# snap-research/graphless-neural-networks

Measured on AMD Instinct MI355X. Metric: aggregated edges/sec (teacher fwd) + student distill steps/sec, ogbn-products 1/2/4/8 GPU, higher is better.
Workload: dtype f32; 1 GPU; ogbn-products-shaped SAGE teacher forward (3 layers 100-256-256-47, BN, layer-wise full-neighbour inference, reference models.py:121-148) + MLP3w8 student KL distillation step; nodes=2449029, nnz=123718280, graph_fingerprint=2449029-123718280-12a892faaf-3b89008b386, parallelism=1 GPU

## Files before the change

graphless-neural-networks_amd/csrc/spmm.hip:

```cpp
#include "glnn_common.h"
#include "source_tail_dev.h"

namespace {

#ifndef GLNN_SPMM_U
#define GLNN_SPMM_U 8
#endif
#ifndef GLNN_FUSED_U
#define GLNN_FUSED_U 8
#endif
#ifndef GLNN_ROWS_PER_WAVE
#define GLNN_ROWS_PER_WAVE 16
#endif
#ifndef GLNN_LONG_ROW
#define GLNN_LONG_ROW 128
#endif
#ifndef GLNN_LONG_BLOCK_ROWS
#define GLNN_LONG_BLOCK_ROWS 512
#endif
#ifndef GLNN_LONG_BLOCK_CAP
#define GLNN_LONG_BLOCK_CAP 512
#endif
constexpr int kBlock = 512;
constexpr int kWavesPerBlock = kBlock / 64;
// ... 283 lines not shown
  const float4 acc = wave_gather_sum<LPR, U, CS, XF>(a.indices, e0, e1, wave, 8, a.x, a.ldx, col4, col_ok, a.col_scale, lane, xf);
  if (lane < LPR && col_ok) st4(a.hub.slab + ((int64_t)sg * 8 + wave) * a.hub.ld_slab + col4, acc);
}

template <int LPR, int U, int MODE, bool CS, int XF = 0>
__device__ __forceinline__ void long_rows_role(const SpmmArgs& a, int lane, int wave, int col4, bool col_ok, const EpCols& ep,
                                               const TailCols& xf) {
  __shared__ int64_t s_rows[kBlock];
  __shared__ int s_count;
  __shared__ float4 s_part[kWavesPerBlock][64];
  const int64_t n_chunks = (a.n_dst + kBlock - 1) / kBlock;
  for (int64_t chunk = blockIdx.x; chunk < n_chunks; chunk += a.n_long_blocks) {
    if (threadIdx.x == 0) s_count = 0;
    __syncthreads();
    const int64_t r = (int64_t)threadIdx.x * n_chunks + chunk;
    if (r < a.n_dst && (a.indptr[r + 1] - a.indptr[r]) > kLongRow) {
      const int slot = atomicAdd(&s_count, 1);
      s_rows[slot] = r;
    }
    __syncthreads();
    const int n_found = s_count;
    for (int i = 0; i < n_found; ++i) {
      const int64_t v = s_rows[i];
      const int64_t e0 = a.indptr[v], e1 = a.indptr[v + 1];
      float4 acc;
      if (e1 - e0 > kHubRow)
        acc = hub_wave_share<LPR, U, CS, XF>(a.hub, a.indices, v, e0, e1, a.x, a.ldx, col4, col_ok, a.col_scale, wave, lane, xf);
      else
        acc = wave_gather_sum<LPR, U, CS, XF>(a.indices, e0, e1, wave, kWavesPerBlock, a.x, a.ldx, col4, col_ok, a.col_scale, lane, xf);
      if (lane < LPR) s_part[wave][lane] = acc;
      __syncthreads();
      if (wave == 0 && lane < LPR && col_ok) {
        float4 t = s_part[0][lane];
#pragma unroll
        for (int w = 1; w < kWavesPerBlock; ++w) t = add4(t, s_part[w][lane]);
        finish_row<MODE, XF>(a, v, e1 - e0, t, col4, ep, xf);
      }
      __syncthreads();
    }
  }
}

template <int LPR, int U, int MODE, bool CS, int XF>
__device__ __forceinline__ void long_rows_role_chunks(const SpmmArgs& a, const ChunkMap& cm, int lane, int wave, int col4, bool col_ok,
                                                      const EpCols& ep, const TailCols& xf) {
  __shared__ int64_t s_rows[kBlock];
  __shared__ int s_count;
  __shared__ float4 s_part[kWavesPerBlock][64];
  int64_t dealt = 0;
#pragma unroll 1
  for (int c = 0; c < cm.n; ++c) {
    const int64_t rs = (int64_t)cm_tile_start(cm, c) * 32;
    int64_t re = (int64_t)cm_tile_start(cm, c + 1) * 32;
    if (re > a.n_dst) re = a.n_dst;
    if (re <= rs) continue;
    const int64_t out_shift = cm_pick(cm.out_shift, c), self_shift = cm_pick(cm.self_shift, c);
    const int64_t n_sub = (re - rs + kBlock - 1) / kBlock;
    const int64_t first = ((int64_t)blockIdx.x - dealt % a.n_long_blocks + a.n_long_blocks) % a.n_long_blocks;
    dealt += n_sub;
#pragma unroll 1
    for (int64_t sub = first; sub < n_sub; sub += a.n_long_blocks) {
      if (threadIdx.x == 0) s_count = 0;
      __syncthreads();
      const int64_t r = rs + (int64_t)threadIdx.x * n_sub + sub;
      if (r < re && (a.indptr[r + 1] - a.indptr[r]) > kLongRow) {
        const int slot = atomicAdd(&s_count, 1);
        s_rows[slot] = r;
      }
      __syncthreads();
      const int n_found = s_count;
      for (int i = 0; i < n_found; ++i) {
        const int64_t v = s_rows[i];
        const int64_t e0 = a.indptr[v], e1 = a.indptr[v + 1];
        float4 acc;
        if (e1 - e0 > kHubRow)
          acc = hub_wave_share<LPR, U, CS, XF>(a.hub, a.indices, v, e0, e1, a.x, a.ldx, col4, col_ok, a.col_scale, wave, lane, xf);
        else
          acc = wave_gather_sum<LPR, U, CS, XF>(a.indices, e0, e1, wave, kWavesPerBlock, a.x, a.ldx, col4, col_ok, a.col_scale, lane, xf);
        if (lane < LPR) s_part[wave][lane] = acc;
        __syncthreads();
        if (wave == 0 && lane < LPR && col_ok) {
          float4 t = s_part[0][lane];
#pragma unroll
          for (int w = 1; w < kWavesPerBlock; ++w) t = add4(t, s_part[w][lane]);
          finish_row<MODE, XF>(a, v, e1 - e0, t, col4, ep, xf, out_shift, self_shift);
        }
        __syncthreads();
      }
    }
    if (wave == 0) {
      asm volatile("s_waitcnt vmcnt(0)" ::: "memory");
      if (lane == 0) {
        const int64_t rpb = a.rows_per_block;
        cm_arrive(cm, c, (int)((re - rs + rpb - 1) / rpb) + a.n_long_blocks);
      }
    }
  }
}

template <int LPR, int U, int MODE, bool CS, int XF = 0, bool CM = false>
__global__ __launch_bounds__(kBlock) void spmm_csr_kernel(const SpmmArgs a0) {
  SpmmArgs a = a0;
  if (gridDim.y > 1) {
    const int off = 256 * (int)blockIdx.y;
    a.x += off; a.out += off; a.d = a0.d - off < 256 ? a0.d - off : 256;
    if (a.x_self) a.x_self += off;
    if (a.ep_scale) a.ep_scale += off;
    if (a.ep_shift) a.ep_shift += off;
  }
  const int lane = threadIdx.x & 63;
  const int wave = __builtin_amdgcn_readfirstlane(threadIdx.x >> 6);
  const int c = lane % LPR;
  const int col4 = c * 4;
  const bool col_ok = col4 < a.d;
  const EpCols ep = load_ep_cols(a, col_ok ? col4 : 0);
  TailCols xf = {};
  if (XF) xf = load_tail_cols(a.xf_scale, a.xf_shift, a.xf_mean, a.xf_rstd, a.xf_thr, a.xf_seed, a.xf_dscale, a.d, col_ok ? col4 : 0, a.xf_on);

  if ((int)blockIdx.x < a.n_long_blocks) {
    if constexpr (CM) long_rows_role_chunks<LPR, U, MODE, CS, XF>(a, a0.cm, lane, wave, col4, col_ok, ep, xf);
    else long_rows_role<LPR, U, MODE, CS, XF>(a, lane, wave, col4, col_ok, ep, xf);
    return;
  }

  __shared__ int s_ticket;
  __shared__ int s_arrived;
  if (threadIdx.x == 0) { s_ticket = 0; if (CM) s_arrived = 0; }
  __syncthreads();
  const int64_t blk = (int64_t)blockIdx.x - a.n_long_blocks;
  const int64_t row_base = blk * a.rows_per_block;
  int chunk = 0;
  int64_t out_shift = 0, self_shift = 0;
  if constexpr (CM) {
#pragma unroll
    for (int c = 1; c < GLNN_MAX_CHUNKS; ++c)
      if (c < a0.cm.n && row_base >= (int64_t)a0.cm.tile_start[c] * 32) chunk = c;
    out_shift = cm_pick(a0.cm.out_shift, chunk);
    self_shift = cm_pick(a0.cm.self_shift, chunk);
  }
#pragma unroll 1
  while (true) {
    int lr = 0;
    if (lane == 0) lr = atomicAdd(&s_ticket, 1);
    lr = __builtin_amdgcn_readfirstlane(lr);
    if (lr >= a.rows_per_block) break;
    const int64_t v = row_base + lr;
    if (v >= a.n_dst) break;
    const int64_t e0 = a.indptr[v], e1 = a.indptr[v + 1];
    const int64_t deg = e1 - e0;
    if (deg > kLongRow) continue;
    float4 acc = wave_gather_sum<LPR, U, CS, XF>(a.indices, e0, e1, 0, 1, a.x, a.ldx, col4, col_ok, a.col_scale, lane, xf);
    if (lane < LPR && col_ok) finish_row<MODE, XF>(a, v, deg, acc, col4, ep, xf, out_shift, self_shift);
  }
  if constexpr (CM) {
    asm volatile("s_waitcnt vmcnt(0)" ::: "memory");
    if (lane == 0 && atomicAdd(&s_arrived, 1) == kWavesPerBlock - 1) {
      const int64_t rs = (int64_t)cm_tile_start(a0.cm, chunk) * 32;
      int64_t re = (int64_t)cm_tile_start(a0.cm, chunk + 1) * 32;
      if (re > a.n_dst) re = a.n_dst;
      const int64_t rpb = a.rows_per_block;
      cm_arrive(a0.cm, chunk, (int)((re - rs + rpb - 1) / rpb) + a.n_long_blocks);
    }
  }
}

constexpr int kShortRows = 4;
constexpr int kShortUnits = 3;
__device__ __forceinline__ int64_t readlane64(int64_t v, int l) {
  const uint32_t lo = (uint32_t)__builtin_amdgcn_readlane((int)(uint32_t)v, l);
  const uint32_t hi = (uint32_t)__builtin_amdgcn_readlane((int)(uint32_t)((uint64_t)v >> 32), l);
  return (int64_t)(((uint64_t)hi << 32) | lo);
}
template <int LPR, int U, int MODE, bool CS, int XF = 0>
__global__ __launch_bounds__(kBlock) void spmm_csr_short_kernel(const SpmmArgs a) {
  constexpr int G = 64 / LPR, RB = kShortRows, UB = kShortUnits;
  const int lane = threadIdx.x & 63;
  const int wave = __builtin_amdgcn_readfirstlane(threadIdx.x >> 6);
  const int c = lane % LPR, g = lane / LPR;
  const int col4 = c * 4;
  const bool col_ok = col4 < a.d;
  const EpCols ep = load_ep_cols(a, col_ok ? col4 : 0);
  TailCols xf = {};
  if (XF) xf = load_tail_cols(a.xf_scale, a.xf_shift, a.xf_mean, a.xf_rstd, a.xf_thr, a.xf_seed, a.xf_dscale, a.d, col_ok ? col4 : 0, a.xf_on);
  if ((int)blockIdx.x < a.n_long_blocks) {
    long_rows_role<LPR, U, MODE, CS, XF>(a, lane, wave, col4, col_ok, ep, xf);
    return;
  }
  __shared__ int s_ticket;
  if (threadIdx.x == 0) s_ticket = 0;
  __syncthreads();
  const int64_t blk = (int64_t)blockIdx.x - a.n_long_blocks;
  const int64_t row_base = blk * a.rows_per_block;
#pragma unroll 1
  while (true) {
    int lr = 0;
    if (lane == 0) lr = atomicAdd(&s_ticket, RB);
    lr = __builtin_amdgcn_readfirstlane(lr);
    if (lr >= a.rows_per_block) break;
    const int64_t v0 = row_base + lr;
    if (v0 >= a.n_dst) break;
    int nr = a.rows_per_block - lr;
    if (nr > RB) nr = RB;
    if (v0 + nr > a.n_dst) nr = (int)(a.n_dst - v0);
    const int64_t my_ptr = a.indptr[v0 + (lane <= nr ? lane : nr)];
    int64_t my_self = v0 + (lane < nr ? lane : 0);
    if (MODE == GLNN_AGG_SAGE_GCN && a.self_rows) my_self = a.self_rows[v0 + (lane < nr ? lane : 0)];
    int64_t e[RB + 1];
#pragma unroll
    for (int r = 0; r <= RB; ++r) e[r] = readlane64(my_ptr, r <= nr ? r : nr);
    const int64_t ebase = e[0];
    int64_t span = e[RB] - ebase;
    const int tot = span < 64 ? (int)span : 64;
    const int my_idx = lane < tot ? ld_idx_stream(a.indices + ebase + lane) : 0;
    float my_cs = 0.f;
    if (CS) my_cs = lane < tot ? a.col_scale[my_idx] : 0.f;
    int hd[RB];
    bool live[RB];
    float4 v[RB][UB], selfv[RB];
    float sc[RB][UB];
    int srcs[RB][UB];
#pragma unroll
    for (int r = 0; r < RB; ++r) {
      const int64_t deg = e[r + 1] - e[r];
      const int off = (int)(e[r] - ebase < 64 ? e[r] - ebase : 64);
      live[r] = r < nr && deg <= kLongRow;
      int h = deg < UB * G ? (int)deg : UB * G;
      if (!live[r] || off + h > tot) h = 0;
      hd[r] = h;
#pragma unroll
      for (int k = 0; k < UB; ++k) {
        const int first = k * G + g;
        const int ei = off + first;
        int src;
        if (G == 1) src = __builtin_amdgcn_readlane(my_idx, ei & 63);
        else src = __shfl(my_idx, ei & 63);
        float cs = 0.f;
        if (CS) cs = (G == 1) ? __builtin_bit_cast(float, __builtin_amdgcn_readlane(__builtin_bit_cast(int, my_cs), ei & 63)) : __shfl(my_cs, ei & 63);
        const bool ok = first < h && col_ok;
        srcs[r][k] = ok ? src : -1;
        sc[r][k] = ok ? cs : 0.f;
        v[r][k] = ok ? ld4(a.x + (int64_t)src * a.ldx + col4) : make_float4(0.f, 0.f, 0.f, 0.f);
      }
      selfv[r] = make_float4(0.f, 0.f, 0.f, 0.f);
      if (MODE == GLNN_AGG_SAGE_GCN) {
        const int64_t sr = readlane64(my_self, r < nr ? r : 0);
        if (live[r] && col_ok) {
          selfv[r] = ld4(a.x_self + sr * a.ld_self + col4);
          if (XF) selfv[r] = tail_apply<XF>(xf, selfv[r], (uint32_t)sr);
        }
      }
    }
#pragma unroll
    for (int r = 0; r < RB; ++r) {
      float4 acc = make_float4(0.f, 0.f, 0.f, 0.f);
#pragma unroll
      for (int k = 0; k < UB; ++k) {
        if (XF) {
          if (srcs[r][k] >= 0) v[r][k] = tail_apply<XF>(xf, v[r][k], (uint32_t)srcs[r][k]);
        }
        acc = CS ? fma4(sc[r][k], v[r][k], acc) : add4(acc, v[r][k]);
      }
      if (!live[r]) continue;
      const int64_t deg = e[r + 1] - e[r];
      if (deg > hd[r])
        acc = wave_gather_acc<LPR, U, CS, XF>(a.indices, e[r] + hd[r], e[r + 1], 0, 1, a.x, a.ldx, col4, col_ok, a.col_scale, lane, xf, acc);
      acc = fold_groups<LPR>(acc);
      if (lane < LPR && col_ok) finish_row_s<MODE>(a, v0 + r, deg, acc, selfv[r], col4, ep);
    }
  }
}

struct DyTail {
  const float* z; int64_t ldz; const float* mean; const float* rstd; const float* a_scale; const float* a_shift;
  uint32_t dthr; uint32_t dseed; float dscale; int relu; float* ws1; float* ws2; int h;
};
struct DyCols { float mu[4], rs[4], sc[4], sf[4]; };
__device__ __forceinline__ DyCols load_dy_cols(const DyTail& t, int col4) {
  DyCols c;
  const float4 mu = ld4(t.mean + col4), rs = ld4(t.rstd + col4), sc = ld4(t.a_scale + col4), sf = ld4(t.a_shift + col4);
  c.mu[0] = mu.x; c.mu[1] = mu.y; c.mu[2] = mu.z; c.mu[3] = mu.w;
  c.rs[0] = rs.x; c.rs[1] = rs.y; c.rs[2] = rs.z; c.rs[3] = rs.w;
  c.sc[0] = sc.x; c.sc[1] = sc.y; c.sc[2] = sc.z; c.sc[3] = sc.w;
  c.sf[0] = sf.x; c.sf[1] = sf.y; c.sf[2] = sf.z; c.sf[3] = sf.w;
  return c;
}
template <bool DROP>
__device__ __forceinline__ void finish_dy_row(const SpmmArgs& a, const DyTail& t, const DyCols& c, int64_t v, float4 acc, float4 z4, int col4,
                                              float (&s1)[4], float (&s2)[4]) {
  const float da[4] = {acc.x, acc.y, acc.z, acc.w}, zz[4] = {z4.x, z4.y, z4.z, z4.w};
  float o[4];
#pragma unroll
  for (int k = 0; k < 4; ++k) {
    float dav = da[k];
    if (DROP) dav = glnn::drop_keep(t.dseed, t.dthr, (uint32_t)v, (uint32_t)(col4 + k)) ? dav * t.dscale : 0.f;
    const float dy = (!t.relu || fmaf(zz[k], c.sc[k], c.sf[k]) > 0.f) ? dav : 0.f;
    s1[k] += dy;
    s2[k] = fmaf(dy, (zz[k] - c.mu[k]) * c.rs[k], s2[k]);
    o[k] = dy;
  }
  st4_stream(a.out + v * a.ldo + col4, make_float4(o[0], o[1], o[2], o[3]));
}

#ifndef GLNN_BN_DY_BATCH
#define GLNN_BN_DY_BATCH 1
#endif
template <int LPR, int U, bool DROP>
__global__ __launch_bounds__(kBlock) void spmm_bn_dy_kernel(const SpmmArgs a, const DyTail t) {
  const int lane = threadIdx.x & 63;
  const int wave = __builtin_amdgcn_readfirstlane(threadIdx.x >> 6);
  const int col4 = (lane % LPR) * 4;
  const bool col_ok = col4 < a.d;
  const DyCols c = load_dy_cols(t, col_ok ? col4 : 0);
  const TailCols xf = {};
  float s1[4] = {0.f, 0.f, 0.f, 0.f}, s2[4] = {0.f, 0.f, 0.f, 0.f};
  __shared__ float4 s_part[kWavesPerBlock][64], s_part2[kWavesPerBlock][64];
  if ((int)blockIdx.x < a.n_long_blocks) {
    __shared__ int64_t s_rows[kBlock], s_sorted[kBlock];
    __shared__ int s_count;
    const int64_t n_chunks = (a.n_dst + kBlock - 1) / kBlock;
    for (int64_t chunk = blockIdx.x; chunk < n_chunks; chunk += a.n_long_blocks) {
      if (threadIdx.x == 0) s_count = 0;
      __syncthreads();
      const int64_t r = (int64_t)threadIdx.x * n_chunks + chunk;
      if (r < a.n_dst && (a.indptr[r + 1] - a.indptr[r]) > kLongRow) s_rows[atomicAdd(&s_count, 1)] = r;
      __syncthreads();
      const int n_found = s_count;
      if ((int)threadIdx.x < n_found) {
        const int64_t mine = s_rows[threadIdx.x];
        int rank = 0;
        for (int i = 0; i < n_found; ++i) rank += s_rows[i] < mine ? 1 : 0;
        s_sorted[rank] = mine;
      }
      __syncthreads();
      for (int i = 0; i < n_found; ++i) {
        const int64_t v = s_sorted[i];
        const int64_t e0 = a.indptr[v], e1 = a.indptr[v + 1];
        float4 z4 = make_float4(0.f, 0.f, 0.f, 0.f);
        if (wave == 0 && lane < LPR && col_ok) z4 = ld4(t.z + v * t.ldz + col4);
        float4 acc;
        if (e1 - e0 > kHubRow) acc = hub_wave_share<LPR, U, true, false>(a.hub, a.indices, v, e0, e1, a.x, a.ldx, col4, col_ok, a.col_scale, wave, lane, xf);
        else acc = wave_gather_sum<LPR, U, true, false>(a.indices, e0, e1, wave, kWavesPerBlock, a.x, a.ldx, col4, col_ok, a.col_scale, lane, xf);
        if (lane < LPR) s_part[wave][lane] = acc;
        __syncthreads();
        if (wave == 0 && lane < LPR && col_ok) {
          float4 sum = s_part[0][lane];
#pragma unroll
          for (int w = 1; w < kWavesPerBlock; ++w) sum = add4(sum, s_part[w][lane]);
          finish_dy_row<DROP>(a, t, c, v, sum, z4, col4, s1, s2);
        }
        __syncthreads();
      }
    }
    if (wave == 0 && lane < LPR && col_ok) {
      st4(t.ws1 + (int64_t)blockIdx.x * t.h + col4, make_float4(s1[0], s1[1], s1[2], s1[3]));
      st4(t.ws2 + (int64_t)blockIdx.x * t.h + col4, make_float4(s2[0], s2[1], s2[2], s2[3]));
    }
    return;
  }
  const int64_t blk = (int64_t)blockIdx.x - a.n_long_blocks;
  const int64_t row_base = blk * a.rows_per_block;
#if GLNN_BN_DY_BATCH
  {
    constexpr int G = 64 / LPR, RB = kShortRows, UB = 2;
    const int g = lane / LPR;
#pragma unroll 1
    for (int lr0 = wave; lr0 < a.rows_per_block; lr0 += kWavesPerBlock * RB) {
      int nr = 0;
#pragma unroll
      for (int r = 0; r < RB; ++r)
        if (lr0 + kWavesPerBlock * r < a.rows_per_block && row_base + lr0 + kWavesPerBlock * r < a.n_dst) nr = r + 1;
      if (nr == 0) break;
      const int rl = (lane >> 1) < nr ? (lane >> 1) : 0;
      const int64_t my_ptr = a.indptr[row_base + lr0 + kWavesPerBlock * rl + (lane & 1)];
      int64_t e0[RB], e1[RB];
      bool live[RB];
      int hd[RB], my_idx[RB];
      float my_cs[RB];
#pragma unroll
      for (int r = 0; r < RB; ++r) {
        e0[r] = readlane64(my_ptr, 2 * r);
        e1[r] = readlane64(my_ptr, 2 * r + 1);
        const int64_t deg = e1[r] - e0[r];
        live[r] = r < nr && deg <= kLongRow;
        hd[r] = live[r] ? (deg < UB * G ? (int)deg : UB * G) : 0;
        my_idx[r] = lane < hd[r] ? ld_idx_stream(a.indices + e0[r] + lane) : 0;
      }
#pragma unroll
      for (int r = 0; r < RB; ++r) my_cs[r] = lane < hd[r] ? a.col_scale[my_idx[r]] : 0.f;
      float4 v[RB][UB], z4[RB];
      float sc[RB][UB];
#pragma unroll
      for (int r = 0; r < RB; ++r) {
        z4[r] = make_float4(0.f, 0.f, 0.f, 0.f);
        if (live[r] && lane < LPR && col_ok) z4[r] = ld4(t.z + (row_base + lr0 + kWavesPerBlock * r) * t.ldz + col4);
#pragma unroll
        for (int k = 0; k < UB; ++k) {
          const int first = k * G + g;
          int src;
          float cs;
          if (G == 1) {
            src = __builtin_amdgcn_readlane(my_idx[r], first & 63);
            cs = __builtin_bit_cast(float, __builtin_amdgcn_readlane(__builtin_bit_cast(int, my_cs[r]), first & 63));
          } else {
            src = __shfl(my_idx[r], first & 63);
            cs = __shfl(my_cs[r], first & 63);
          }
          const bool ok = first < hd[r] && col_ok;
          sc[r][k] = ok ? cs : 0.f;
          v[r][k] = ok ? ld4(a.x + (int64_t)src * a.ldx + col4) : make_float4(0.f, 0.f, 0.f, 0.f);
        }
      }
#pragma unroll
      for (int r = 0; r < RB; ++r) {
        if (!live[r]) continue;
        float4 acc = make_float4(0.f, 0.f, 0.f, 0.f);
#pragma unroll
        for (int k = 0; k < UB; ++k) acc = fma4(sc[r][k], v[r][k], acc);
        if (e1[r] - e0[r] > hd[r])
          acc = wave_gather_acc<LPR, U, true, false>(a.indices, e0[r] + hd[r], e1[r], 0, 1, a.x, a.ldx, col4, col_ok, a.col_scale, lane, xf, acc);
        acc = fold_groups<LPR>(acc);
        if (lane < LPR && col_ok) finish_dy_row<DROP>(a, t, c, row_base + lr0 + kWavesPerBlock * r, acc, z4[r], col4, s1, s2);
      }
    }
  }
#else
#pragma unroll 1
  for (int lr = wave; lr < a.rows_per_block; lr += kWavesPerBlock) {
    const int64_t v = row_base + lr;
    if (v >= a.n_dst) break;
    const int64_t e0 = a.indptr[v], e1 = a.indptr[v + 1];
    if (e1 - e0 > kLongRow) continue;
    float4 z4 = make_float4(0.f, 0.f, 0.f, 0.f);
    if (lane < LPR && col_ok) z4 = ld4(t.z + v * t.ldz + col4);
    const float4 acc = wave_gather_sum<LPR, U, true, false>(a.indices, e0, e1, 0, 1, a.x, a.ldx, col4, col_ok, a.col_scale, lane, xf);
    if (lane < LPR && col_ok) finish_dy_row<DROP>(a, t, c, v, acc, z4, col4, s1, s2);
  }
#endif
  if (lane < LPR) {
    s_part[wave][lane] = make_float4(s1[0], s1[1], s1[2], s1[3]);
    s_part2[wave][lane] = make_float4(s2[0], s2[1], s2[2], s2[3]);
  }
  __syncthreads();
  if (wave == 0 && lane < LPR && col_ok) {
    float4 u = s_part[0][lane], w2 = s_part2[0][lane];
#pragma unroll
    for (int w = 1; w < kWavesPerBlock; ++w) { u = add4(u, s_part[w][lane]); w2 = add4(w2, s_part2[w][lane]); }
    st4(t.ws1 + (int64_t)blockIdx.x * t.h + col4, u);
    st4(t.ws2 + (int64_t)blockIdx.x * t.h + col4, w2);
  }
}

struct LnDzTail {
  const float* z; int64_t ldz; const float* mean; const float* rstd; const float* gamma; const float* beta;
  uint32_t dthr; uint32_t dseed; float dscale; float inv_h; float* ws; int h;
};
__device__ __forceinline__ float wave_sum64(float v) {
#pragma unroll
  for (int o = 32; o > 0; o >>= 1) v += __shfl_xor(v, o);
  return v;
}
template <bool DROP>
__device__ __forceinline__ void finish_ln_row(const SpmmArgs& a, const LnDzTail& t, const float (&g)[4], const float (&b)[4], int64_t v, float4 acc,
                                              float4 z4, int col4, bool mine, float (&pg)[4], float (&pb)[4], float (&pz)[4]) {
  const float mu = t.mean[v], rs = t.rstd[v];
  const float da[4] = {acc.x, acc.y, acc.z, acc.w}, zz[4] = {z4.x, z4.y, z4.z, z4.w};
  float xh[4], dy[4], dxh[4];
  float s1 = 0.f, s2 = 0.f;
#pragma unroll
  for (int k = 0; k < 4; ++k) {
    float x = 0.f, d = 0.f;
    if (mine && col4 + k < t.h) {
      x = (zz[k] - mu) * rs;
      d = da[k];
      if (DROP) d = glnn::drop_keep(t.dseed, t.dthr, (uint32_t)v, (uint32_t)(col4 + k)) ? d * t.dscale : 0.f;
      if (!(fmaf(x, g[k], b[k]) > 0.f)) d = 0.f;
    }
    xh[k] = x;
    dy[k] = d;
    dxh[k] = d * g[k];
    s1 += dxh[k];
    s2 = fmaf(dxh[k], x, s2);
  }
  const float m1 = wave_sum64(s1) * t.inv_h, m2 = wave_sum64(s2) * t.inv_h;
  if (!mine) return;
  float o[4];
#pragma unroll
  for (int k = 0; k < 4; ++k) {
    o[k] = col4 + k < t.h ? rs * (dxh[k] - m1 - xh[k] * m2) : 0.f;
    pg[k] = fmaf(dy[k], xh[k], pg[k]);
    pb[k] += dy[k];
    pz[k] += o[k];
  }
  st4_stream(a.out + v * a.ldo + col4, make_float4(o[0], o[1], o[2], o[3]));
}

template <int LPR, int U, bool DROP>
__global__ __launch_bounds__(kBlock) void spmm_ln_dz_kernel(const SpmmArgs a, const LnDzTail t) {
  const int lane = threadIdx.x & 63;
  const int wave = __builtin_amdgcn_readfirstlane(threadIdx.x >> 6);
  const int col4 = (lane % LPR) * 4;
  const bool col_ok = col4 < a.d;
  const bool mine = lane < LPR && col_ok;
  float g[4], b[4];
#pragma unroll
  for (int k = 0; k < 4; ++k) {
    const bool ok = col_ok && col4 + k < a.d;
    g[k] = ok ? t.gamma[col4 + k] : 0.f;
    b[k] = ok ? t.beta[col4 + k] : 0.f;
  }
  const TailCols xf = {};
  float pg[4] = {0.f, 0.f, 0.f, 0.f}, pb[4] = {0.f, 0.f, 0.f, 0.f}, pz[4] = {0.f, 0.f, 0.f, 0.f};
  __shared__ float4 s_part[kWavesPerBlock][64];
  if ((int)blockIdx.x < a.n_long_blocks) {
    __shared__ int64_t s_rows[kBlock], s_sorted[kBlock];
    __shared__ int s_count;
    const int64_t n_chunks = (a.n_dst + kBlock - 1) / kBlock;
    for (int64_t chunk = blockIdx.x; chunk < n_chunks; chunk += a.n_long_blocks) {
      if (threadIdx.x == 0) s_count = 0;
      __syncthreads();
      const int64_t r = (int64_t)threadIdx.x * n_chunks + chunk;
      if (r < a.n_dst && (a.indptr[r + 1] - a.indptr[r]) > kLongRow) s_rows[atomicAdd(&s_count, 1)] = r;
      __syncthreads();
      const int n_found = s_count;
      if ((int)threadIdx.x < n_found) {
        const int64_t me = s_rows[threadIdx.x];
        int rank = 0;
        for (int i = 0; i < n_found; ++i) rank += s_rows[i] < me ? 1 : 0;
        s_sorted[rank] = me;
      }
      __syncthreads();
      for (int i = 0; i < n_found; ++i) {
        const int64_t v = s_sorted[i];
        const int64_t e0 = a.indptr[v], e1 = a.indptr[v + 1];
        float4 z4 = make_float4(0.f, 0.f, 0.f, 0.f);
        if (wave == 0 && mine) z4 = ld4(t.z + v * t.ldz + col4);
        float4 acc;
        if (e1 - e0 > kHubRow) acc = hub_wave_share<LPR, U, true, 0>(a.hub, a.indices, v, e0, e1, a.x, a.ldx, col4, col_ok, a.col_scale, wave, lane, xf);
        else acc = wave_gather_sum<LPR, U, true, 0>(a.indices, e0, e1, wave, kWavesPerBlock, a.x, a.ldx, col4, col_ok, a.col_scale, lane, xf);
        if (lane < LPR) s_part[wave][lane] = acc;
        __syncthreads();
        if (wave == 0) {
          float4 sum = make_float4(0.f, 0.f, 0.f, 0.f);
          if (lane < LPR) {
            sum = s_part[0][lane];
#pragma unroll
            for (int w = 1; w < kWavesPerBlock; ++w) sum = add4(sum, s_part[w][lane]);
          }
          finish_ln_row<DROP>(a, t, g, b, v, sum, z4, col4, mine, pg, pb, pz);
        }
        __syncthreads();
      }
    }
  } else {
    const int64_t row_base = ((int64_t)blockIdx.x - a.n_long_blocks) * a.rows_per_block;
#pragma unroll 1
    for (int lr = wave; lr < a.rows_per_block; lr += kWavesPerBlock) {
      const int64_t v = row_base + lr;
      if (v >= a.n_dst) break;
      const int64_t e0 = a.indptr[v], e1 = a.indptr[v + 1];
      if (e1 - e0 > kLongRow) continue;
      float4 z4 = make_float4(0.f, 0.f, 0.f, 0.f);
      if (mine) z4 = ld4(t.z + v * t.ldz + col4);
      const float4 acc = wave_gather_sum<LPR, U, true, 0>(a.indices, e0, e1, 0, 1, a.x, a.ldx, col4, col_ok, a.col_scale, lane, xf);
      finish_ln_row<DROP>(a, t, g, b, v, acc, z4, col4, mine, pg, pb, pz);
    }
  }
  float* slot = t.ws + (int64_t)blockIdx.x * 3 * t.h;
#pragma unroll
  for (int q = 0; q < 3; ++q) {
    const float* p = q == 0 ? pg : (q == 1 ? pb : pz);
    __syncthreads();
    if (lane < LPR) s_part[wave][lane] = make_float4(p[0], p[1], p[2], p[3]);
    __syncthreads();
    if (wave == 0 && mine) {
      float4 u = s_part[0][lane];
#pragma unroll
      for (int w = 1; w < kWavesPerBlock; ++w) u = add4(u, s_part[w][lane]);
      const float uu[4] = {u.x, u.y, u.z, u.w};
#pragma unroll
      for (int k = 0; k < 4; ++k)
        if (col4 + k < t.h) slot[q * t.h + col4 + k] = uu[k];
    }
  }
}

typedef float f32x16 __attribute__((ext_vector_type(16)));
constexpr int kFusedWaves = 8;
constexpr int kFusedBlock = 64 * kFusedWaves;

template <bool CM>
__device__ __forceinline__ void store_out(float* p, float v) {
  *p = v;
}

template <bool CM>
__device__ __forceinline__ void chunk_arrive(const ChunkMap& cm, int chunk, bool stored, int lane, int* s_arrived) {
  if constexpr (CM) {
    if (stored) asm volatile("s_waitcnt vmcnt(0)" ::: "memory");
    if (lane != 0) return;
    if (atomicAdd(s_arrived, 1) != kFusedWaves - 1) return;
    int* cnt = cm.arrivals + chunk;
    const int prev = __hip_atomic_fetch_add(cnt, 1, __ATOMIC_RELAXED, __HIP_MEMORY_SCOPE_AGENT);
    int expected = 0;
    uint32_t* sig = nullptr;
#pragma unroll
    for (int c = 0; c < GLNN_MAX_CHUNKS; ++c)
      if (c == chunk) { expected = cm.tile_start[c + 1] - cm.tile_start[c]; sig = cm.signal[c]; }
    if (prev == expected - 1) {
      __hip_atomic_store(cnt, 0, __ATOMIC_RELAXED, __HIP_MEMORY_SCOPE_AGENT);
      __hip_atomic_store(sig, cm.epoch, __ATOMIC_RELEASE, __HIP_MEMORY_SCOPE_SYSTEM);
    }
  }
}

struct FusedArgs {
  const int64_t* indptr; const int32_t* indices; int64_t n_dst;
  const float* x; int64_t ldx; int d_in;
  const float* x_self; int64_t ld_self;
  const float* w_packed; int d_out; int kgroups;
  const float* ep_scale; const float* ep_shift; int relu;
  float* out; int64_t ldo;
  const float* w2_packed; int d_out2; int kgroups2; float* out2; int64_t ldo2;
  const int32_t* tile_order;
  HubPlan hub;
  ChunkMap cm;
  float* agg_out; const float* agg_in; int64_t ld_agg;
};

constexpr int kAggNone = 0, kAggOut = 1, kAggIn = 2;

template <int LPR, int U, int RT, bool CM = false, int AGG = kAggNone>
__global__ __launch_bounds__(kFusedBlock) void sage_fused_kernel(const FusedArgs a) {
  constexpr int kFusedRows = 32 * RT;
  extern __shared__ __attribute__((aligned(16))) float lds_a[];
  __shared__ float4 s_part[kFusedWaves / 2][64];
  const int lane = threadIdx.x & 63;
  const int wave = __builtin_amdgcn_readfirstlane(threadIdx.x >> 6);
  const int col4 = (lane % LPR) * 4;
  const bool col_ok = col4 < a.d_in;
  const int kpad = a.kgroups * 8;
  const int lda = kpad + 4;
  const int tile_id = (AGG != kAggIn && a.tile_order) ? a.tile_order[blockIdx.x] : (int)blockIdx.x;
  const int64_t row0 = (int64_t)tile_id * kFusedRows;
  int chunk = 0;
  int64_t self_shift = 0, out_shift = 0;
  if constexpr (CM) {
    self_shift = a.cm.self_shift[0];
    out_shift = a.cm.out_shift[0];
#pragma unroll
    for (int c = 1; c < GLNN_MAX_CHUNKS; ++c)
      if (c < a.cm.n && tile_id >= a.cm.tile_start[c]) { chunk = c; self_shift = a.cm.self_shift[c]; out_shift = a.cm.out_shift[c]; }
  }

  __shared__ int s_next;
  __shared__ int s_arrived;
  if constexpr (AGG == kAggIn) {
    const int kv = kpad / 4, dpad = (a.d_in + 3) & ~3;
    for (int i = threadIdx.x; i < kFusedRows * kv; i += kFusedBlock) {
      const int lr = i / kv, c4 = (i - lr * kv) * 4;
      const int64_t v = row0 + lr;
      float4 y = make_float4(0.f, 0.f, 0.f, 0.f);
      if (v < a.n_dst && c4 < dpad) y = ld4_stream(a.agg_in + v * a.ld_agg + c4);
      st4(lds_a + lr * lda + c4, y);
    }
// ... 713 lines not shown
```

Baseline: 15.58 billion edges/s.

## Software-pipeline indptr and index loads in BN-dy SpMM short-row batch path

Adds a new default batch mode for the BN backward dy SpMM kernel. It prefetches the next batch's indptr values and neighbour indices, and the indptr for the batch after that, while the current batch's feature gathers and accumulation run. The goal is to hide the latency of dependent index loads. It also sets an occupancy hint of 4 waves per EU. The extra live prefetch state adds register pressure, and the occupancy hint may cause spills or limit occupancy.

New measurement: 15.58 billion edges/s. About the same (-0.0%).

```diff
diff --git a/graphless-neural-networks_amd/csrc/spmm.hip b/graphless-neural-networks_amd/csrc/spmm.hip
--- a/graphless-neural-networks_amd/csrc/spmm.hip
+++ b/graphless-neural-networks_amd/csrc/spmm.hip
@@ -609,10 +609,15 @@
 }
 
 #ifndef GLNN_BN_DY_BATCH
-#define GLNN_BN_DY_BATCH 1
+#define GLNN_BN_DY_BATCH 2
+#endif
+#if GLNN_BN_DY_BATCH == 2
+#define GLNN_BN_DY_BOUNDS __launch_bounds__(kBlock) __attribute__((amdgpu_waves_per_eu(4)))
+#else
+#define GLNN_BN_DY_BOUNDS __launch_bounds__(kBlock)
 #endif
 template <int LPR, int U, bool DROP>
-__global__ __launch_bounds__(kBlock) void spmm_bn_dy_kernel(const SpmmArgs a, const DyTail t) {
+__global__ GLNN_BN_DY_BOUNDS void spmm_bn_dy_kernel(const SpmmArgs a, const DyTail t) {
   const int lane = threadIdx.x & 63;
   const int wave = __builtin_amdgcn_readfirstlane(threadIdx.x >> 6);
   const int col4 = (lane % LPR) * 4;
@@ -666,7 +671,108 @@
   }
   const int64_t blk = (int64_t)blockIdx.x - a.n_long_blocks;
   const int64_t row_base = blk * a.rows_per_block;
-#if GLNN_BN_DY_BATCH
+#if GLNN_BN_DY_BATCH == 2
+  {
+    constexpr int G = 64 / LPR, RB = kShortRows, UB = 2, STEP = kWavesPerBlock * RB;
+    constexpr int UC = U < 4 / G ? U : 4 / G;
+    const int g = lane / LPR;
+    const auto rows_of = [&](int lr0) {
+      int nr = 0;
+#pragma unroll
+      for (int r = 0; r < RB; ++r)
+        if (lr0 + kWavesPerBlock * r < a.rows_per_block && row_base + lr0 + kWavesPerBlock * r < a.n_dst) nr = r + 1;
+      return nr;
+    };
+    const auto ptr_of = [&](int lr0, int nr) -> int64_t {
+      const int rl = (lane >> 1) < nr ? (lane >> 1) : 0;
+      return nr > 0 ? a.indptr[row_base + lr0 + kWavesPerBlock * rl + (lane & 1)] : (int64_t)0;
+    };
+    const auto decode = [&](int64_t ptr, int nr, int64_t (&e0)[RB], int64_t (&e1)[RB], bool (&live)[RB], int (&hd)[RB]) {
+#pragma unroll
+      for (int r = 0; r < RB; ++r) {
+        e0[r] = readlane64(ptr, 2 * r);
+        e1[r] = readlane64(ptr, 2 * r + 1);
+        const int64_t deg = e1[r] - e0[r];
+        live[r] = r < nr && deg <= kLongRow;
+        hd[r] = live[r] ? (deg < UB * G ? (int)deg : UB * G) : 0;
+      }
+    };
+    constexpr int W = UB * G;
+    const int pr = lane / W, pj = lane % W;
+    const auto packed_ok = [&](const int (&hd)[RB]) {
+      int h = 0;
+#pragma unroll
+      for (int r = 0; r < RB; ++r)
+        if (pr == r) h = hd[r];
+      return pj < h;
+    };
+    const auto idx_of = [&](const int64_t (&e0)[RB], const int (&hd)[RB]) {
+      int64_t base = 0;
+#pragma unroll
+      for (int r = 0; r < RB; ++r)
+        if (pr == r) base = e0[r];
+      return packed_ok(hd) ? ld_idx_stream(a.indices + base + pj) : 0;
+    };
+    int lr0 = wave;
+    int nr = rows_of(lr0);
+    int64_t e0[RB], e1[RB];
+    bool live[RB];
+    int hd[RB];
+    decode(ptr_of(lr0, nr), nr, e0, e1, live, hd);
+    int nr_n = rows_of(lr0 + STEP);
+    int64_t ptr_n = ptr_of(lr0 + STEP, nr_n);
+    int my_idx = idx_of(e0, hd);
+    float my_cs = packed_ok(hd) ? a.col_scale[my_idx] : 0.f;
+#pragma unroll 1
+    while (nr > 0) {
+      int64_t f0[RB], f1[RB];
+      bool live_n[RB];
+      int hd_n[RB];
+      decode(ptr_n, nr_n, f0, f1, live_n, hd_n);
+      float4 v[RB][UB], z4[RB];
+#pragma unroll
+      for (int r = 0; r < RB; ++r) {
+        z4[r] = make_float4(0.f, 0.f, 0.f, 0.f);
+        if (live[r] && lane < LPR && col_ok) z4[r] = ld4(t.z + (row_base + lr0 + kWavesPerBlock * r) * t.ldz + col4);
+#pragma unroll
+        for (int k = 0; k < UB; ++k) {
+          const int first = k * G + g;
+          int src;
+          if (G == 1) src = __builtin_amdgcn_readlane(my_idx, r * W + k);
+          else src = __shfl(my_idx, r * W + first);
+          v[r][k] = first < hd[r] && col_ok ? ld4(a.x + (int64_t)src * a.ldx + col4) : make_float4(0.f, 0.f, 0.f, 0.f);
+        }
+      }
+      const int idx_n = idx_of(f0, hd_n);
+      const int nr_nn = rows_of(lr0 + 2 * STEP);
+      const int64_t ptr_nn = ptr_of(lr0 + 2 * STEP, nr_nn);
+#pragma unroll
+      for (int r = 0; r < RB; ++r) {
+        if (!live[r]) continue;
+        float4 acc = make_float4(0.f, 0.f, 0.f, 0.f);
+#pragma unroll
+        for (int k = 0; k < UB; ++k) {
+          const int first = k * G + g;
+          float cs;
+          if (G == 1) cs = __builtin_bit_cast(float, __builtin_amdgcn_readlane(__builtin_bit_cast(int, my_cs), r * W + k));
+          else cs = __shfl(my_cs, r * W + first);
+          acc = fma4(first < hd[r] && col_ok ? cs : 0.f, v[r][k], acc);
+        }
+        if (e1[r] - e0[r] > hd[r])
+          acc = wave_gather_acc<LPR, UC, true, false>(a.indices, e0[r] + hd[r], e1[r], 0, 1, a.x, a.ldx, col4, col_ok, a.col_scale, lane, xf, acc);
+        acc = fold_groups<LPR>(acc);
+        if (lane < LPR && col_ok) finish_dy_row<DROP>(a, t, c, row_base + lr0 + kWavesPerBlock * r, acc, z4[r], col4, s1, s2);
+      }
+      my_cs = packed_ok(hd_n) ? a.col_scale[idx_n] : 0.f;
+      my_idx = idx_n;
+#pragma unroll
+      for (int r = 0; r < RB; ++r) {
+        e0[r] = f0[r]; e1[r] = f1[r]; live[r] = live_n[r]; hd[r] = hd_n[r];
+      }
+      nr = nr_n; nr_n = nr_nn; ptr_n = ptr_nn; lr0 += STEP;
+    }
+  }
+#elif GLNN_BN_DY_BATCH
   {
     constexpr int G = 64 / LPR, RB = kShortRows, UB = 2;
     const int g = lane / LPR;
```
